# HuiGuanLab/Lite-MKD

Hardware: AMD Instinct MI355X
Metric: episodes/sec (5-way 5-shot, 8x224^2 frames) (higher is better)
Workload: dtype f32

## Files before the change

include/lmkd.h:

```cpp
#ifndef LMKD_H
#define LMKD_H
#ifdef __cplusplus
extern "C" {
#endif

int lmkd_abi_version(void);
const char* lmkd_last_error(void);
int lmkd_device_check(int device);
int lmkd_set_activation_dtype(int mode);
int lmkd_get_activation_dtype(void);

int lmkd_gemm_f32(char layA, char layB, int M, int N, int K, float alpha, const float* A, long lda, long sA,
                  const float* B, long ldb, long sB, float beta, float* C, long ldc, long sC, const float* bias,
                  int relu, int batch, void* stream);
int lmkd_gemm_set_mode(int mode);
int lmkd_gemm_set_tile(int t);
long lmkd_gemm_ticket_words(void);
int lmkd_gemm_f32_splitk(char layA, char layB, int M, int N, int K, float alpha, const float* A, long lda, long sA,
                         const float* B, long ldb, long sB, float beta, float* C, long ldc, long sC, const float* bias,
                         int relu, int batch, void* workspace, long ws_bytes, unsigned* tickets, void* stream);

long lmkd_conv2d_packed_weight_elems(int Cout, int Cin, int Cs, int KH, int KW, int mode);
int lmkd_conv2d_pack_weights(const float* w_oihw, float* wp, int Cout, int Cin, int Cs, int KH, int KW, int mode ,
                             void* stream);
// ... 5 lines not shown
  const void* x_words;
  const void* dy_words;
  void* out_words;
  const void* ref_words;
  int flags;
} lmkd_amax_desc;
#define LMKD_AMAX_FENCED 1
int lmkd_h2_fence_eval(const void* const* words, void* const* refs, int n, int* flags, void* stream);
long lmkd_conv_h2_fallbacks(void);
int lmkd_amax(const float* x, long n, void* word, void* stream);
long lmkd_amax_words(void);
long lmkd_conv2d_plane_elems(int ncols, int Kp);
long lmkd_conv_h2_launches(void);
int lmkd_conv2d_repack_multi(const float* const* ws, void* const* wfs, const int* dims, int n, void* stream);
int lmkd_conv2d_split_weights(const float* wp, void* wf, int ncols, int Kp, void* stream);
int lmkd_conv_get_compute_dtype(void);
int lmkd_conv_set_wgrad_planes(int on);
int lmkd_conv_set_patch(int on);
int lmkd_conv_set_stem_patch(int on);
int lmkd_conv_set_s2_patch(int on);
int lmkd_conv_set_wgrad_win16(int on);
int lmkd_conv_set_wgrad_stem(int on);
int lmkd_conv_set_wgrad_window(int on);
int lmkd_conv_set_patch16(int on);
int lmkd_conv_set_persistent(int on);
int lmkd_conv_set_xcd_mode(int mode);
int lmkd_conv_set_tile(int id);
int lmkd_conv2d_fwd(const float* x, const float* wp_fwd, float* y, float* stat_partial, int N, int H, int W, int Cs, int Cout,
                    int KH, int KW, int stride, int pad, void* stream);
int lmkd_conv2d_fwd_pre(const float* x_raw, const float* pre_stats, const float* wp_fwd, float* y, float* stat_partial, int N, int H,
                        int W, int Cs, int Cout, int KH, int KW, int stride, int pad, void* stream);
int lmkd_conv2d_fwd_bn(const float* x, const float* wp_fwd, float* y, const float* bn_stats, const float* res , int relu,
                       int N, int H, int W, int Cs, int Cout, int KH, int KW, int stride, int pad, void* stream,
                       const lmkd_amax_desc* amax );
int lmkd_conv2d_bwd_data(const float* dy, const float* wp_dgrad, float* dx, int N, int H, int W, int Cin, int Cout, int KH, int KW,
                         int stride, int pad, int accumulate, void* stream);
int lmkd_conv2d_bwd_data_bn_tiles(int N, int H, int W, int Cin, int Cout, int KH, int KW, int stride, int pad);
int lmkd_conv2d_bwd_data_bn(const float* dy, const float* wp_dgrad, float* dx, const float* bn_x, const float* bn_stats, float* part,
                            int N, int H, int W, int Cin, int Cout, int KH, int KW, int stride, int pad, void* stream);
long lmkd_conv2d_bwd_weight_workspace(int N, int H, int W, int Cs, int Cout, int KH, int KW, int stride, int pad);
int lmkd_conv2d_bwd_weight(const float* x, const float* dy, float* dw_oihw, float* workspace, long ws_bytes, int N, int H, int W,
                           int Cs, int Cin, int Cout, int KH, int KW, int stride, int pad, void* stream);
int lmkd_conv2d_bwd_weight_pre(const float* x_raw, const float* pre_stats, const float* dy, float* dw_oihw, float* workspace,
                               long ws_bytes, int N, int H, int W, int Cs, int Cin, int Cout, int KH, int KW, int stride, int pad,
                               void* stream);

// ... 182 lines not shown
```

lite-mkd_amd/csrc/conv.hip:

```cpp
#include "gemm_core.h"
#include <atomic>
#include <mutex>

struct ConvGemmArgs {
  const float* src;
  const float* wpk;
  float* out;
  float* stat_partial;
  int N, Hs, Ws, Cs;
  int Hr, Wr, rows_per_class, tiles_per_class;
  int sh;
  int Ho, Wo, Co, omul;
  int Kp, cps, nclass;
  int n_rt, n_ct, xcd_mode;
  int taps_pm1;
  int grid_step;
  int grid_total;
  int same;
  int halo;
  int accum;
  const float* ep_stats;
  const float* ep_res;
  int ep_relu;
  const float* pre_stats;
// ... 1362 lines not shown
}
extern "C" int lmkd_conv2d_bwd_data_bn(const float* dy, const float* wd, float* dx, const float* bn_x, const float* bn_stats, float* part,
                                       int N, int H, int W, int Cin, int Cout, int KH, int KW, int stride, int pad, void* stream) {
  LMKD_REQUIRE(dy && wd && dx && bn_x && bn_stats && part, "lmkd_conv2d_bwd_data_bn: null pointer");
  LMKD_REQUIRE(aligned16(dy) && aligned16(wd) && aligned16(bn_x) && aligned16(bn_stats), "lmkd_conv2d_bwd_data_bn: operands must be 16-byte aligned");
  ConvGemmArgs a;
  if (const int rc = bwd_data_args(a, dy, wd, dx, N, H, W, Cin, Cout, KH, KW, stride, pad, 0)) return rc;
  a.bnb_x = bn_x; a.bnb_stats = bn_stats; a.stat_partial = part;
  const ConvPlan p = plan_dgrad(a);
  LMKD_REQUIRE(p.bnb_form, "lmkd_conv2d_bwd_data_bn: this launch has no fused form (lmkd_conv2d_bwd_data_bn_tiles returned 0)");
  return launch_conv(a, p, (hipStream_t)stream);
}

static int g_wgrad_planes = 1;
extern "C" int lmkd_conv_set_wgrad_planes(int on) { g_wgrad_planes = on ? 1 : 0; return LMKD_OK; }
static int g_wgrad_win16 = 1;
extern "C" int lmkd_conv_set_wgrad_win16(int on) { g_wgrad_win16 = on ? 1 : 0; return LMKD_OK; }
static int g_wgrad_window = 1;
extern "C" int lmkd_conv_set_wgrad_window(int on) { g_wgrad_window = on < 0 ? 0 : on; return LMKD_OK; }
static inline bool wgrad_win_eligible(int W, int Cs, int Cout, int KH, int KW, int stride, int pad) {
  return g_wgrad_window && g_wgrad_planes && conv_planes() && KH == 3 && KW == 3 && stride == 1 && pad == 1 &&
         Cs % 32 == 0 && 32 + 2 * (W + 1) <= 256;
}
static void wgrad_win_plan(int Mpix, int W, int Cs, int Cout, int* cob, int* splits, int* steps_per_split) {
  *cob = Cout >= 128 ? 4 : 2;
  const int tiles = cdiv(Cout, 32 * *cob) * (Cs / 32);
  const int steps = cdiv(Mpix, LMKD_BK);
  const int warm = cdiv(2 * (W + 1), LMKD_BK);
  const int resident = 256 * ((conv_nprod() >= 6 && *cob == 2) ? 2 : 8 / *cob);
  int sp = g_wgrad_window > 1 ? cdiv(g_wgrad_window, tiles)
                              : std::max((int)(((long)resident * steps + 19600L * 4 / *cob) / (39200L * 4 / *cob)), cdiv(128, tiles));
  const int cap = std::max(1, steps / (12 * warm));
  if (sp > cap) sp = cap;
  *steps_per_split = cdiv(steps, sp);
  *splits = cdiv(steps, *steps_per_split);
}

static void wgrad_plan(int Mpix, int Cout, int Kp, int* splits, int* steps_per_split, int* bm, int* bn, bool planes = false) {
  *bm = Cout <= 64 ? 64 : 128;
  *bn = (Kp % 128 == 0 && Kp >= 1024) ? 128 : 64;
  int per_cu = (*bm == 128 && *bn == 128) ? 2 : ((*bm == 64 && *bn == 64) ? 4 : 3);
  if (planes) {
    if (*bm == 64 && *bn == 128) *bn = 64;
    const int npl = conv_nprod() == 1 ? 1 : 3;
    const long lds = 1L * npl * LMKD_BK * ((*bm * 2 + 64) + (*bn * 2 + 64));
    per_cu = (int)(160 * 1024 / lds);
    if (per_cu > 4) per_cu = 4;
    if (per_cu < 1) per_cu = 1;
  }
  const int tiles = cdiv(Cout, *bm) * cdiv(Kp, *bn);
  const int steps = cdiv(Mpix, LMKD_BK);
  const int slots = 256 * per_cu;
  int best_sp = 1;
  double best_cost = 1e30;
// ... 8 lines not shown
    if (cost < best_cost) { best_cost = cost; best_sp = sp; }
  }
  if (planes && *bm == 64 && *bn == 64 && best_sp < cdiv(steps, 64)) best_sp = cdiv(steps, 64);
  *steps_per_split = cdiv(steps, best_sp);
  *splits = cdiv(steps, *steps_per_split);
}

static int g_wgrad_stem = 1;
extern "C" int lmkd_conv_set_wgrad_stem(int on) { g_wgrad_stem = on ? 1 : 0; return LMKD_OK; }
static int stem_wgrad_plan(int N, int H, int W, int Cs, int Cout, int KH, int KW, int stride, int pad, int* G) {
  if (!g_wgrad_stem || !g_wgrad_planes || conv_nprod(g_lmkd_act_bf16) < 6 || Cs != 4 || Cout != 64 || KH != 7 || KW != 7 || stride != 2 || pad != 3) return 0;
  const int Ho = conv_out(H, KH, stride, pad), Wo = conv_out(W, KW, stride, pad);
  if (Wo < 17 || Wo > 128 || W > 2 * Wo || Ho < 1) return 0;
  const int units = N * cdiv(Ho, 2);
  int g = std::max(1, 2048 / (2 * Wo));
  g = std::min(g, std::max(1, units / 256));
  *G = g;
  return cdiv(units, g);
}

enum class WgFam : unsigned char {
  Stem,
  Win16,
  Win,
  Planes,
  Tile,
};
struct WgradPlan {
  WgFam fam;
  bool pre, act16, smallc;
  int nprod;
  int bm, bn;
  int cob;
  int G;
  int splits, splits0, sps0, sps1, seg_pix0;
  int xcd;
  int grid;
  long need;
  long ws;
};

static long wgrad_workspace(int N, int H, int W, int Cs, int Cout, int KH, int KW, int stride, int pad) {
  const int Ho = conv_out(H, KH, stride, pad), Wo = conv_out(W, KW, stride, pad);
  const int Kp = KH * kw_padded(Cs, KW) * Cs;
  int G, splits, sps, bm, bn;
  if (const int slabs = stem_wgrad_plan(N, H, W, Cs, Cout, KH, KW, stride, pad, &G)) return (long)slabs * Cout * Kp * sizeof(float);
  wgrad_plan(N * Ho * Wo, Cout, Kp, &splits, &sps, &bm, &bn, conv_planes() && g_wgrad_planes);
  if (wgrad_win_eligible(W, Cs, Cout, KH, KW, stride, pad)) {
    int cob, wsplits, wsps;
    wgrad_win_plan(N * Ho * Wo, W, Cs, Cout, &cob, &wsplits, &wsps);
    splits = std::max(splits, wsplits);
  }
  return (long)splits * Cout * Kp * sizeof(float);
}

static WgradPlan plan_wgrad(int N, int H, int W, int Cs, int Cout, int KH, int KW, int stride, int pad, int seg_n0, bool pre, bool maxima) {
  WgradPlan p;
  memset(&p, 0, sizeof(p));
  const bool act16 = g_lmkd_act_bf16;
  const int Ho = conv_out(H, KH, stride, pad), Wo = conv_out(W, KW, stride, pad);
  const int Kp = KH * kw_padded(Cs, KW) * Cs, Mpix = N * Ho * Wo;
  p.pre = pre; p.act16 = act16; p.smallc = Cs == 4;
  p.ws = wgrad_workspace(N, H, W, Cs, Cout, KH, KW, stride, pad);
  if (seg_n0)
    p.ws = std::max(p.ws, wgrad_workspace(seg_n0, H, W, Cs, Cout, KH, KW, stride, pad) + wgrad_workspace(N - seg_n0, H, W, Cs, Cout, KH, KW, stride, pad));
  p.seg_pix0 = seg_n0 ? seg_n0 * Ho * Wo : Mpix;
  if (const int slabs = stem_wgrad_plan(N, H, W, Cs, Cout, KH, KW, stride, pad, &p.G)) {
    p.fam = WgFam::Stem;
    p.nprod = conv_nprod(false, maxima);
    p.splits = p.grid = slabs;
  } else if (wgrad_win_eligible(W, Cs, Cout, KH, KW, stride, pad)) {
    const bool w16 = g_wgrad_win16 && conv_nprod(act16) >= 6;
    p.fam = w16 ? WgFam::Win16 : WgFam::Win;
    p.nprod = w16 ? conv_nprod(false, maxima) : conv_nprod(act16);
    wgrad_win_plan(Mpix, W, Cs, Cout, &p.cob, &p.splits, &p.sps0);
    p.splits0 = p.splits;
    if (seg_n0) {
      int sp1, cob1;
      wgrad_win_plan(p.seg_pix0, W, Cs, Cout, &p.cob, &p.splits0, &p.sps0);
      wgrad_win_plan(Mpix - p.seg_pix0, W, Cs, Cout, &cob1, &sp1, &p.sps1);
      p.splits = p.splits0 + sp1;
    }
    p.grid = 8 * cdiv(p.splits, 8) * cdiv(Cout, 32 * p.cob) * (Cs / 32);
  } else {
    const bool planes = conv_planes() && g_wgrad_planes;
    p.fam = planes ? WgFam::Planes : WgFam::Tile;
    p.nprod = planes ? conv_nprod(act16, maxima && !p.smallc && !pre) : (conv_nprod() == 1 ? 1 : 0);
    wgrad_plan(Mpix, Cout, Kp, &p.splits, &p.sps0, &p.bm, &p.bn, planes);
    p.splits0 = p.splits;
    if (seg_n0) {
      int sp1, bm1, bn1;
      wgrad_plan(p.seg_pix0, Cout, Kp, &p.splits0, &p.sps0, &p.bm, &p.bn, planes);
      wgrad_plan(Mpix - p.seg_pix0, Cout, Kp, &sp1, &p.sps1, &bm1, &bn1, planes);
      p.splits = p.splits0 + sp1;
    }
    p.xcd = (g_xcd_mode != 0 && g_xcd_mode != 1 && p.splits >= 32) ? 1 : 0;
    p.grid = (p.xcd ? 8 * cdiv(p.splits, 8) : p.splits) * cdiv(Cout, p.bm) * cdiv(Kp, p.bn);
  }
  p.need = (long)p.splits * Cout * Kp * sizeof(float);
  return p;
}

template <int NPROD, int D, int RLC>
static void launch_stem_wgrad(const StemWgradArgs& w, dim3 grid, size_t lds, hipStream_t s) {
  lds_attr_once<stem_wgrad_kernel<NPROD, D, RLC>>(160 * 1024);
  hipLaunchKernelGGL((stem_wgrad_kernel<NPROD, D, RLC>), grid, dim3(512), lds, s, w);
}
template <int NPROD>
static void launch_stem_wgrad(const StemWgradArgs& w, dim3 grid, size_t lds, hipStream_t s) {
  const bool deep = cdiv(2 * w.Wo, 32) >= 6;
  if (deep && w.RL == 1856) launch_stem_wgrad<NPROD, 6, 1856>(w, grid, lds, s);
  else if (deep) launch_stem_wgrad<NPROD, 6, 0>(w, grid, lds, s);
  else launch_stem_wgrad<NPROD, 2, 0>(w, grid, lds, s);
}
template <int COB>
static void launch_wgrad_win(const WgradWinArgs& w, const WgradPlan& p, bool big, hipStream_t s) {
  const dim3 grid(p.grid);
  if (p.fam == WgFam::Win16) {
    constexpr int JW = COB == 2 ? 1 : 2;
    constexpr int NT = 64 * COB * (2 / JW);
    with_nprod<3, 6, 9>(p.nprod, [&](auto np) {
      if (big && p.pre) hipLaunchKernelGGL((conv_wgrad_win16_kernel<COB, np, 256, true, 9, JW>), grid, dim3(NT), 0, s, w);
      else if (big) hipLaunchKernelGGL((conv_wgrad_win16_kernel<COB, np, 256, false, 9, JW>), grid, dim3(NT), 0, s, w);
      else if (p.pre) hipLaunchKernelGGL((conv_wgrad_win16_kernel<COB, np, 128, true, 9, JW>), grid, dim3(NT), 0, s, w);
      else hipLaunchKernelGGL((conv_wgrad_win16_kernel<COB, np, 128, false, 9, JW>), grid, dim3(NT), 0, s, w);
    });
    return;
  }
  auto go = [&](auto np, auto a16, auto pre) {
    constexpr int NPROD = decltype(np)::value;
    constexpr bool A16 = decltype(a16)::value, PRE = decltype(pre)::value;
    constexpr int TPW = (COB == 2 && NPROD != 1) ? 5 : 9;
    constexpr int NT = 64 * COB * ((9 + TPW - 1) / TPW);
    if (big) hipLaunchKernelGGL((conv_wgrad_win_kernel<COB, NPROD, A16, 256, PRE, TPW>), grid, dim3(NT), 0, s, w);
    else hipLaunchKernelGGL((conv_wgrad_win_kernel<COB, NPROD, A16, 128, PRE, TPW>), grid, dim3(NT), 0, s, w);
  };
  using T = std::true_type;
  using F = std::false_type;
  if (p.act16) go(std::integral_constant<int, 1>{}, T{}, F{});
  else with_nprod<1, 6, 9>(p.nprod, [&](auto np) { if (p.pre) go(np, F{}, T{}); else go(np, F{}, F{}); });
// ... 44 lines not shown
  LMKD_REQUIRE(ws_bytes >= p.need, "lmkd_conv2d_bwd_weight: workspace too small");
  hipStream_t s = (hipStream_t)stream;
  if (p.fam == WgFam::Stem) {
    LMKD_REQUIRE((long)Mpix * 64 * 4 < 0xffffffe0L && (long)N * H * W * 16 < 0xffffffe0L, "lmkd_conv2d_bwd_weight: tensor too large for 32-bit byte offsets");
    StemWgradArgs w;
    memset(&w, 0, sizeof(w));
    w.dy = dy; w.x = x; w.slab = workspace;
    w.h2_xw = amax_x; w.h2_dyw = amax_dy;
    w.N = N; w.H = H; w.W = W; w.Ho = Ho; w.Wo = Wo;
    w.upi = cdiv(Ho, 2); w.units = N * w.upi; w.G = p.G; w.slabs = p.splits;
    w.RL = 16 * Wo + 64;
    const size_t lds = (size_t)2 * 10 * 3 * w.RL + 2 * 3 * STEM_WG_APLANE;
    with_nprod<3, 6, 9>(p.nprod, [&](auto np) { launch_stem_wgrad<np>(w, dim3(p.grid), lds, s); });
    LMKD_CHECK_LAUNCH("stem_wgrad_kernel");
    if (Kp <= 256) {
      hipLaunchKernelGGL(wgrad_reduce_stem_kernel, dim3(Cout), dim3(256, 4), 0, s, (const float*)workspace, dw_oihw, p.splits, Cout, Cin, Cs, KH, KW,
                         KWp, Kp, accumulate);
    } else {
      launch_wgrad_reduce((const float*)workspace, dw_oihw, p.splits, Cout, Cin, Cs, KH, KW, KWp, Kp, accumulate, s);
    }
    LMKD_CHECK_LAUNCH("wgrad_reduce_kernel");
    return LMKD_OK;
  }
  if (p.fam == WgFam::Win16 || p.fam == WgFam::Win) {
    LMKD_REQUIRE((long)Mpix * std::max(Cs, Cout) * 4 < 2147483647L, "lmkd_conv2d_bwd_weight: tensor too large for 32-bit byte offsets");
    WgradWinArgs w;
    memset(&w, 0, sizeof(w));
    w.dy = dy; w.x = x; w.slab = workspace; w.pre_stats = pre_stats;
    w.h2_xw = amax_x; w.h2_dyw = amax_dy;
    w.N = N; w.H = H; w.W = W; w.Cs = Cs; w.Co = Cout; w.Kp = Kp; w.Mpix = Mpix;
    w.steps_total = cdiv(Mpix, LMKD_BK);
    w.splits = p.splits; w.steps_per_split = p.sps0;
    w.seg_pix0 = p.seg_pix0; w.seg_splits0 = p.splits0; w.sps1 = p.sps1;
    w.n_ct = cdiv(Cout, 32 * p.cob); w.n_it = Cs / 32;
    w.div_hw = make_fastdiv(H * W); w.div_w = make_fastdiv(W);
    const bool big = 32 + 2 * (W + 1) > 128;
    if (p.cob == 4) launch_wgrad_win<4>(w, p, big, s);
    else launch_wgrad_win<2>(w, p, big, s);
    LMKD_CHECK_LAUNCH("conv_wgrad_win_kernel");
    launch_wgrad_reduce((const float*)workspace, dw_oihw, p.splits, Cout, Cin, Cs, KH, KW, KWp, Kp, accumulate, s);
    LMKD_CHECK_LAUNCH("wgrad_reduce_kernel");
    return LMKD_OK;
  }
  WgradArgs a;
  memset(&a, 0, sizeof(a));
  a.dy = dy; a.x = x; a.slab = workspace; a.pre_stats = pre_stats;
  a.h2_xw = amax_x; a.h2_dyw = amax_dy;
  a.N = N; a.Hs = H; a.Ws = W; a.Cs = Cs;
  a.Ho = Ho; a.Wo = Wo; a.Co = Cout;
  a.stride = stride; a.pad = pad; a.KH = KH; a.KW = KW; a.KWp = KWp;
  a.Kp = Kp; a.Mpix = Mpix;
  a.steps_per_split = p.sps0;
  a.seg_pix0 = p.seg_pix0; a.seg_splits0 = p.splits0; a.sps1 = p.sps1;
  a.steps_total = cdiv(Mpix, LMKD_BK);
  a.div_hw = make_fastdiv(Ho * Wo); a.div_w = make_fastdiv(Wo);
  a.n_mt = cdiv(Cout, p.bm); a.n_jt = cdiv(Kp, p.bn); a.splits = p.splits;
  a.xcd_mode = p.xcd;
  const int bm = p.bm, bn = p.bn;
  LMKD_REQUIRE(!smallc || (bm == 64 && bn == 64), "lmkd_conv2d_bwd_weight: padded-stem path expects Cout <= 64");
// ... 39 lines not shown
extern "C" int lmkd_conv2d_bwd_weight_acc(const float* x, const float* pre_stats, const float* dy, float* dw_oihw, float* workspace,
                                          long ws_bytes, int N, int H, int W, int Cs, int Cin, int Cout, int KH, int KW, int stride,
                                          int pad, void* stream) {
  return conv2d_bwd_weight_impl(x, pre_stats, dy, dw_oihw, workspace, ws_bytes, N, H, W, Cs, Cin, Cout, KH, KW, stride, pad, stream, 1);
}


extern "C" int lmkd_conv2d_bwd_weight_seg(const float* x, const float* pre_stats, const float* dy, float* dw_oihw, float* workspace, long ws_bytes,
                                          int N, int H, int W, int Cs, int Cin, int Cout, int KH, int KW, int stride, int pad, int accumulate,
                                          int seg_n0, void* stream, const lmkd_amax_desc* amax) {
  return conv2d_bwd_weight_impl(x, pre_stats, dy, dw_oihw, workspace, ws_bytes, N, H, W, Cs, Cin, Cout, KH, KW, stride, pad, stream, accumulate, seg_n0, amax);
}

extern "C" int lmkd_conv2d_plan(int kind, int N, int H, int W, int Cs, int Cin, int Cout, int KH, int KW, int stride, int pad,
                                int* info) {
  LMKD_REQUIRE(info && kind >= 0 && kind <= 2, "lmkd_conv2d_plan: kind must be 0 (forward), 1 (data gradient) or 2 (weight gradient)");
  LMKD_REQUIRE(N > 0 && H > 0 && W > 0 && Cout > 0 && KH > 0 && KW > 0 && stride > 0, "lmkd_conv2d_plan: bad shape");
  if (kind == 2) {
    const WgradPlan p = plan_wgrad(N, H, W, Cs, Cout, KH, KW, stride, pad, 0, false, false);
    info[1] = p.xcd; info[2] = p.splits; info[3] = p.grid;
    switch (p.fam) {
      case WgFam::Stem: info[0] = 14; info[4] = 2; break;
      case WgFam::Win16:
      case WgFam::Win: info[0] = p.cob == 4 ? 5 : 6; info[1] = 1; info[4] = 1; break;
      default: info[0] = (p.bm == 128 && p.bn == 128) ? 1 : (p.bm == 128 ? 2 : (p.bn == 128 ? 4 : 3)); info[4] = 0; break;
    }
    return LMKD_OK;
  }
  ConvGemmArgs a;
  if (kind == 0) fwd_geometry(a, N, H, W, Cs, Cout, KH, KW, stride, pad, 0);
  else dgrad_geometry(a, N, H, W, Cin, Cout, KH, KW, stride, pad, 0);
  const ConvPlan p = kind == 0 ? plan_fwd(a, KH, KW, pad) : plan_dgrad(a);
  info[0] = p.tile; info[1] = p.xcd; info[2] = p.nclass; info[3] = p.grid;
  info[4] = p.fam == ConvFam::Stem ? 2 : (p.fam == ConvFam::Patch || p.fam == ConvFam::Patch16 || p.fam == ConvFam::Patch1p ? 1 : 0);
  return LMKD_OK;
}
```

lite-mkd_amd/csrc/wgrad_win.h:

```cpp
#pragma once

struct WgradWinArgs {
  const float* dy;
  const float* x;
  float* slab;
  const float* pre_stats;
  int N, H, W, Cs, Co, Kp;
  int Mpix, steps_total, steps_per_split, splits;
  int n_ct, n_it;
  int seg_pix0, seg_splits0, sps1;
  FastDiv div_hw, div_w;
  const unsigned* h2_xw;
  const unsigned* h2_dyw;
};
template <int COB, int NPROD, bool ACT16, int R, bool PRE = false, int TPW = 9>
__global__ __launch_bounds__(64 * COB * ((9 + TPW - 1) / TPW)) void conv_wgrad_win_kernel(WgradWinArgs a) {
  constexpr int NPL = NPROD == 1 ? 1 : 3;
  static_assert(!ACT16 || (NPROD == 1 && !PRE), "bf16 tensors: one plane, no store-side arithmetic");
  constexpr int THREADS = 64 * COB * ((9 + TPW - 1) / TPW), BM = 32 * COB;
  constexpr int LDA = BM * 2 + 64, A_PLANE = LMKD_BK * LDA;
  constexpr int LDX = 64, X_PLANE = (R + 1) * LDX;
  constexpr int ESZ = ACT16 ? 2 : 4, EPL = ACT16 ? 8 : 4;
  constexpr int A_LPR = BM / EPL, A_RPP = THREADS / A_LPR, A_NI = (LMKD_BK + A_RPP - 1) / A_RPP;
  constexpr int X_LPR = 32 / EPL, X_RPP = THREADS / X_LPR, X_NI = (LMKD_BK + X_RPP - 1) / X_RPP;
  static_assert(THREADS % A_LPR == 0 && THREADS % X_LPR == 0 && (LDA / 64) % 2 == 1, "tile layout");
  __shared__ __attribute__((aligned(16))) unsigned char s_dy[NPL * A_PLANE];
  __shared__ __attribute__((aligned(16))) unsigned char s_x[NPL * X_PLANE];
  __shared__ __attribute__((aligned(16))) unsigned s_adr[2][9 * LMKD_BK];
  const int tid = threadIdx.x, lane = tid & 63, wave = tid >> 6;
  const int tiles = a.n_ct * a.n_it;
// ... 144 lines not shown
            c = __builtin_amdgcn_mfma_f32_32x32x16_bf16(fa[g][1], fb[0], c, 0, 0, 0);
            c = __builtin_amdgcn_mfma_f32_32x32x16_bf16(fa[g][0], fb[0], c, 0, 0, 0);
          }
        }
        acc[ti] = c;
      }
      __syncthreads();
    }
  }

  float* C = a.slab + (long)z * a.Co * a.Kp;
#pragma unroll
  for (int ti = 0; ti < TPW; ++ti) {
    if (9 % TPW != 0 && tap0 + ti >= 9) break;
    const int col = (tap0 + ti) * a.Cs + ci0 + (lane & 31);
#pragma unroll
    for (int e = 0; e < 16; ++e) {
      const int row = co0 + cw * 32 + acc_row(e, lane);
      if (row < a.Co) C[(long)row * a.Kp + col] = acc[ti][e];
    }
  }
}

template <int COB, int NPROD, int R, bool PRE = false, int TPW = 9, int JW = 2>
__global__ __launch_bounds__(64 * COB * ((9 + TPW - 1) / TPW) * (2 / JW), JW == 2 ? 2 : 3) void conv_wgrad_win16_kernel(WgradWinArgs a) {
  static_assert(JW == 2 || (JW == 1 && TPW == 9), "the channel-block split exists for nine taps per wave");
  static_assert(NPROD == 6 || NPROD == 9 || NPROD == 3, "three bf16 planes (6 / 9 products) or two fp16 planes (3 products: conv_patch16.h)");
  constexpr int NPL = NPROD == 3 ? 2 : 3;
  constexpr int THREADS = 64 * COB * ((9 + TPW - 1) / TPW) * (2 / JW), BM = 32 * COB;
  constexpr int LDA = BM * 2 + 32, A_PLANE = LMKD_BK * LDA;
  constexpr int LDX = 64, X_PLANE = (R + 1) * LDX;
  constexpr int A_LPR = BM / 4, A_RPP = THREADS / A_LPR, A_NI = (LMKD_BK + A_RPP - 1) / A_RPP;
  constexpr int X_LPR = 8, X_RPP = THREADS / X_LPR, X_NI = (LMKD_BK + X_RPP - 1) / X_RPP;
  static_assert(THREADS % A_LPR == 0 && THREADS % X_LPR == 0 && (LDA / 32) % 2 == 1, "tile layout");
  __shared__ __attribute__((aligned(16))) unsigned char s_dy[NPL * A_PLANE];
  __shared__ __attribute__((aligned(16))) unsigned char s_x[NPL * X_PLANE];
  __shared__ __attribute__((aligned(16))) unsigned s_adr[2][9 * LMKD_BK];
  const int tid = threadIdx.x, lane = tid & 63, wave = tid >> 6;
  const int tiles = a.n_ct * a.n_it;
  const int xj = blockIdx.x >> 3;
  const int z = (blockIdx.x & 7) + 8 * (xj / tiles);
  if (z >= a.splits) return;
  const int tz = xj - (xj / tiles) * tiles;
  const int co0 = (tz % a.n_ct) * BM, ci0 = (tz / a.n_ct) * 32;
  const WinSlab sl = win_slab(z, a.Mpix, a.steps_per_split, a.seg_pix0, a.seg_splits0, a.sps1);
  const int nk = sl.nk, kend = sl.kend;
  const int halo = a.W + 1;

  const __amdgpu_buffer_rsrc_t rs_dy = x3_rsrc(a.dy, (long)a.Mpix * a.Co * 4);
  const __amdgpu_buffer_rsrc_t rs_x = x3_rsrc(a.x, (long)a.Mpix * a.Cs * 4);
  const int a_c = (tid % A_LPR) * 4, a_r = tid / A_LPR;
  const bool a_cin = co0 + a_c < a.Co;
  const int x_c = (tid % X_LPR) * 4, x_r = tid / X_LPR;
  u32x4 ra[A_NI], rx[X_NI];
  unsigned x_ok = 0;
  float h2_sx = 1.f, h2_sdy = 1.f;
  if constexpr (NPROD == 3) {
    h2_sx = h2_scale(amax_read(a.h2_xw, sl.seg));
    h2_sdy = h2_scale(amax_read(a.h2_dyw, sl.seg));
  }
  float4 psc = float4(), psh = float4();
  if (PRE) {
    psc = *reinterpret_cast<const float4*>(a.pre_stats + (long)sl.seg * 5 * a.Cs + 2 * a.Cs + ci0 + x_c);
    psh = *reinterpret_cast<const float4*>(a.pre_stats + (long)sl.seg * 5 * a.Cs + 3 * a.Cs + ci0 + x_c);
  }
  auto load_dy = [&](int k0) {
#pragma unroll
    for (int i = 0; i < A_NI; ++i) {
      const int p = k0 + a_r + A_RPP * i;
      ra[i] = __builtin_amdgcn_raw_buffer_load_b128(rs_dy, (a_cin && a_r + A_RPP * i < LMKD_BK && p < kend) ? (unsigned)((p * a.Co + co0 + a_c) * 4) : X3_OOB, 0, 0);
    }
  };
  auto load_x = [&](int q0) {
#pragma unroll
    for (int i = 0; i < X_NI; ++i) {
      const int q = q0 + x_r + X_RPP * i;
      const bool ok = x_r + X_RPP * i < LMKD_BK && q >= 0 && q < a.Mpix;
      rx[i] = __builtin_amdgcn_raw_buffer_load_b128(rs_x, ok ? (unsigned)((q * a.Cs + ci0 + x_c) * 4) : X3_OOB, 0, 0);
      if (PRE) x_ok = ok ? (x_ok | (1u << i)) : (x_ok & ~(1u << i));
    }
  };
  auto as_f4 = [](const u32x4& r) { return make_float4(__uint_as_float(r.x), __uint_as_float(r.y), __uint_as_float(r.z), __uint_as_float(r.w)); };
  auto store_dy = [&]() {
#pragma unroll
    for (int i = 0; i < A_NI; ++i) {
      if (a_r + A_RPP * i >= LMKD_BK) continue;
      if constexpr (NPROD == 3) {
        uint2 p0, p1;
        h2_split4(as_f4(ra[i]), h2_sdy, p0, p1);
        unsigned char* d = s_dy + (a_r + A_RPP * i) * LDA + a_c * 2;
        *reinterpret_cast<uint2*>(d) = p0;
        *reinterpret_cast<uint2*>(d + A_PLANE) = p1;
      } else {
        tr_store4<NPL, LDA, A_PLANE>(s_dy, a_r + A_RPP * i, a_c, as_f4(ra[i]));
      }
    }
  };
  auto store_x = [&](int q0) {
#pragma unroll
    for (int i = 0; i < X_NI; ++i) {
      if (x_r + X_RPP * i >= LMKD_BK) continue;
      const int slot = (q0 + x_r + X_RPP * i) & (R - 1);
      float4 v = as_f4(rx[i]);
      if (PRE && ((x_ok >> i) & 1u)) {
        v.x = fmaxf(fmaf(v.x, psc.x, psh.x), 0.f); v.y = fmaxf(fmaf(v.y, psc.y, psh.y), 0.f);
        v.z = fmaxf(fmaf(v.z, psc.z, psh.z), 0.f); v.w = fmaxf(fmaf(v.w, psc.w, psh.w), 0.f);
      }
      uint2 p0, p1, p2;
      if constexpr (NPROD == 3) h2_split4(v, h2_sx, p0, p1); else x3_split4(v, p0, p1, p2);
      unsigned char* d = s_x + slot * LDX + ((x_c * 2) ^ (((slot >> 2) & 1) << 5));
      *reinterpret_cast<uint2*>(d) = p0;
      *reinterpret_cast<uint2*>(d + X_PLANE) = p1;
      if constexpr (NPL == 3) *reinterpret_cast<uint2*>(d + 2 * X_PLANE) = p2;
    }
  };
  auto fill_adr = [&](unsigned* tab, int k0) {
    for (int e = tid; e < 9 * LMKD_BK; e += THREADS) {
      const int tp = e >> 5, r = e & 31;
      const int p = k0 + r;
      unsigned adr = (unsigned)(R * LDX);
      if (p < kend) {
        const int n = fdiv(p, a.div_hw);
        const int rem = p - n * a.H * a.W;
        const int h = fdiv(rem, a.div_w), w = rem - h * a.W;
        const int dh = tp / 3 - 1, dw = tp - (tp / 3) * 3 - 1;
        if ((unsigned)(h + dh) < (unsigned)a.H && (unsigned)(w + dw) < (unsigned)a.W) {
          const int slot = (p + dh * a.W + dw) & (R - 1);
          adr = (unsigned)(slot * LDX + (((slot >> 2) & 1) << 5));
        }
      }
      tab[tp * LMKD_BK + (r & 15) * 2 + (r >> 4)] = adr;
    }
  };

  const int q4 = lane >> 4, idx = lane & 15;
  const int cw = wave % COB, tap0 = JW == 2 ? (wave / COB) * TPW : 0, j0 = JW == 2 ? 0 : wave / COB;
  const int offA = (4 * q4 + (idx >> 2)) * LDA + (cw * 32 + 4 * (idx & 3)) * 2;
  const unsigned cbx = (unsigned)(8 * (idx & 3));
  f32x4 acc[TPW][2][JW];
#pragma unroll
  for (int t = 0; t < TPW; ++t)
#pragma unroll
    for (int i = 0; i < 2; ++i)
#pragma unroll
      for (int j = 0; j < JW; ++j) acc[t][i][j] = f32x4{0.f, 0.f, 0.f, 0.f};

  if (nk > 0) {
    const int kfirst = sl.kfirst;
    for (int j = tid; j < NPL * LDX / 4; j += THREADS)
      reinterpret_cast<unsigned*>(s_x + (j / (LDX / 4)) * X_PLANE + R * LDX)[j % (LDX / 4)] = 0u;
    for (int q0 = kfirst - halo; q0 < kfirst + halo; q0 += LMKD_BK) {
      load_x(q0);
      store_x(q0);
    }
    fill_adr(s_adr[0], kfirst);
    load_dy(kfirst);
    load_x(kfirst + halo);
    for (int t = 0; t < nk; ++t) {
      const int k0 = kfirst + t * LMKD_BK;
      store_dy();
      store_x(k0 + halo);
      __syncthreads();
      if (t + 1 < nk) {
        load_dy(k0 + LMKD_BK);
        load_x(k0 + LMKD_BK + halo);
        fill_adr(s_adr[(t + 1) & 1], k0 + LMKD_BK);
      }
      bf16x8 fa[2][NPL];
#pragma unroll
      for (int i = 0; i < 2; ++i)
#pragma unroll
        for (int p = 0; p < NPL; ++p) {
          const unsigned char* ap = s_dy + p * A_PLANE + offA + i * 32;
          const s16x4_t lo = __builtin_amdgcn_ds_read_tr16_b64_v4i16((s16x4_t __attribute__((address_space(3)))*)ap);
          const s16x4_t hi = __builtin_amdgcn_ds_read_tr16_b64_v4i16((s16x4_t __attribute__((address_space(3)))*)(ap + 16 * LDA));
          union { s16x4_t s[2]; bf16x8 b; } u;
          u.s[0] = lo; u.s[1] = hi;
          fa[i][p] = u.b;
        }
      if constexpr (NPROD == 3 && JW == 2) {
        static_assert(NPROD != 3 || TPW == 9, "all nine taps per wave");
        auto read_fb = [&](int tp, bf16x8 (&fb)[JW][NPL]) {
          const uint2 a2 = *reinterpret_cast<const uint2*>(&s_adr[t & 1][tp * LMKD_BK + (4 * q4 + (idx >> 2)) * 2]);
#pragma unroll
          for (int j = 0; j < JW; ++j) {
            const unsigned lo_a = (a2.x ^ (unsigned)((j0 + j) << 5)) + cbx, hi_a = (a2.y ^ (unsigned)((j0 + j) << 5)) + cbx;
#pragma unroll
            for (int p = 0; p < NPL; ++p) {
// ... 111 lines not shown
```

lite-mkd_amd/ops.py:

```python
import ctypes
import os
import itertools
import math

import torch

from ._lib import lib
from . import _audit


def _raw_stream(device_index=None):
    return torch._C._cuda_getCurrentRawStream(torch._C._cuda_getDevice() if device_index is None else device_index)


def _stream():
    return ctypes.c_void_p(_raw_stream())


def _p(t):
    if t is None:
        return None
    if _audit.ON:
        _audit.note(t)
    return ctypes.c_void_p(t.data_ptr())
# ... 24 lines not shown


def _f32(x):
    return ctypes.c_float(float(x))


def _empty(shape, like):
    return torch.empty(shape, dtype=torch.float32, device=like.device)


_ACT_DTYPE = [torch.float32]


def set_activation_dtype(name):
    modes = {"fp32": (0, torch.float32), "bf16": (1, torch.bfloat16)}
    if name not in modes:
        raise ValueError(name)
    lib().call("lmkd_set_activation_dtype", modes[name][0])
    _ACT_DTYPE[0] = modes[name][1]


def get_activation_dtype():
    return "bf16" if _ACT_DTYPE[0] is torch.bfloat16 else "fp32"


def _empty_act(shape, like):
    return torch.empty(shape, dtype=_ACT_DTYPE[0], device=like.device)


def gemm(layA, layB, M, N, K, A, lda, B, ldb, C, ldc, alpha=1.0, beta=0.0, bias=None, relu=False,
         batch=1, sA=0, sB=0, sC=0, A_off=0, B_off=0, C_off=0, split_k=None):
    _chk(A, B, C, bias)
    es = 4
    if _audit.ON:
        for t in (A, B, C):
            _audit.note(t)
    if GEMM_SPLIT_K if split_k is None else split_k:
        ws, tk = _gemm_workspace(C)
        lib().call("lmkd_gemm_f32_splitk", layA.encode(), layB.encode(), M, N, K, _f32(alpha),
                   ctypes.c_void_p(A.data_ptr() + A_off * es), lda, sA,
                   ctypes.c_void_p(B.data_ptr() + B_off * es), ldb, sB, _f32(beta),
                   ctypes.c_void_p(C.data_ptr() + C_off * es), ldc, sC, _p(bias), int(relu), batch, _p(ws), ws.numel(), _p(tk), _stream())
        return C
    lib().call("lmkd_gemm_f32", layA.encode(), layB.encode(), M, N, K, _f32(alpha),
               ctypes.c_void_p(A.data_ptr() + A_off * es), lda, sA,
               ctypes.c_void_p(B.data_ptr() + B_off * es), ldb, sB, _f32(beta),
# ... 2719 lines not shown
```

lite-mkd_amd/schedule.py:

```python
import contextlib
import dataclasses
import os


_PIPELINE = [False]


@dataclasses.dataclass
class Schedule:
    conv_dtype: str = "fp32x3"
    act_dtype: str = "fp32"
    overlap_trunk_calls: bool = True
    merge_trunk_calls: bool = False
    pipeline_episodes: bool = False
    side_wgrad: bool = True
    sync_wgrad_at_backward_end: bool = False
    teacher_stream: bool = True
    heads_on_two_streams: bool = True
    side_linear_wgrad: bool = True
    direct_param_grad: bool = True
    repack_at_step: bool = True
    fuse_two_head_linear: bool = True
    dgrad_bn_stats: bool = True
    stem_pooled_bwd: bool = True
    pre_in_plane_modes: bool = True
    fuse_pre_all_modes: bool = False
    trx_proj_on_conv: bool = False
    gemm_split_k: bool = False

    @classmethod
    def bench(cls, **over):
        kw = dict(merge_trunk_calls=True, pipeline_episodes=True)
        kw.update(over)
        return cls(**kw)

    @classmethod
    def two_call(cls, **over):
        return cls(**over)

    @classmethod
    def serial(cls, **over):
        kw = dict(overlap_trunk_calls=False, merge_trunk_calls=False, side_wgrad=False, sync_wgrad_at_backward_end=True, teacher_stream=False,
                  heads_on_two_streams=False, side_linear_wgrad=False, direct_param_grad=False, repack_at_step=False, pipeline_episodes=False)
        kw.update(over)
        return cls(**kw)

    @classmethod
    def from_env(cls, env=None, **over):
        env = os.environ if env is None else env
        names = {"overlap_trunk_calls": "LMKD_OVERLAP", "merge_trunk_calls": "LMKD_MERGE", "pipeline_episodes": "LMKD_PIPELINE", "side_wgrad": "LMKD_SIDE_WGRAD",
                 "sync_wgrad_at_backward_end": "LMKD_SYNC_WG", "teacher_stream": "LMKD_TEACHER_STREAM", "heads_on_two_streams": "LMKD_HEADS2",
                 "side_linear_wgrad": "LMKD_SIDE_LINEAR", "direct_param_grad": "LMKD_DIRECT_GRAD", "repack_at_step": "LMKD_REPACK",
                 "fuse_two_head_linear": "LMKD_FC_FUSED", "dgrad_bn_stats": "LMKD_DGRAD_BN", "stem_pooled_bwd": "LMKD_STEM_POOLED",
                 "pre_in_plane_modes": "LMKD_PRE_X3", "fuse_pre_all_modes": "LMKD_FUSE_PRE", "trx_proj_on_conv": "LMKD_TRX_CONV",
                 "gemm_split_k": "LMKD_GEMM_SPLIT"}
        s = cls.bench(**over)
        for field, var in names.items():
            if var in env and field not in over:
                setattr(s, field, env[var] == "1")
        return s

    _WHERE = {
        "overlap_trunk_calls": ("model.backbone.resnet", "OVERLAP_TRUNK_CALLS"), "merge_trunk_calls": ("model.backbone.resnet", "MERGE_TRUNK_CALLS"),
        "side_wgrad": ("ops", "SIDE_WGRAD"), "sync_wgrad_at_backward_end": ("ops", "SYNC_WGRAD_AT_BACKWARD_END"),
        "teacher_stream": ("trainloop", "TEACHER_STREAM"), "heads_on_two_streams": ("ops", "HEADS_ON_TWO_STREAMS"),
        "side_linear_wgrad": ("ops", "SIDE_LINEAR_WGRAD"), "direct_param_grad": ("ops", "DIRECT_PARAM_GRAD"),
        "repack_at_step": ("trainloop", "REPACK_AT_STEP"), "fuse_two_head_linear": ("ops", "FUSE_TWO_HEAD_LINEAR"),
        "dgrad_bn_stats": ("ops", "DGRAD_BN_STATS"), "stem_pooled_bwd": ("ops", "STEM_POOLED_BWD"),
        "pre_in_plane_modes": ("ops", "PRE_IN_PLANE_MODES"), "fuse_pre_all_modes": ("ops", "FUSE_PRE_ALL_MODES"),
        "trx_proj_on_conv": ("ops", "TRX_PROJ_ON_CONV"), "gemm_split_k": ("ops", "GEMM_SPLIT_K"),
    }

    def _targets(self):
        import importlib
        pkg = __name__.rsplit(".", 1)[0]
        for field, (mod, attr) in self._WHERE.items():
            yield field, importlib.import_module(pkg + "." + mod), attr

    def apply(self, arithmetic=True):
        from . import ops
        for field, mod, attr in self._targets():
            setattr(mod, attr, bool(getattr(self, field)))
        _PIPELINE[0] = bool(self.pipeline_episodes)
        if arithmetic:
            ops.set_conv_compute_dtype(self.conv_dtype)
            ops.set_activation_dtype(self.act_dtype)
        return self

    @classmethod
    def current(cls):
        from . import ops
        s = cls(conv_dtype=ops.get_conv_compute_dtype(), act_dtype=ops.get_activation_dtype(), pipeline_episodes=_PIPELINE[0])
        for field, mod, attr in s._targets():
            setattr(s, field, bool(getattr(mod, attr)))
        return s

    @contextlib.contextmanager
    def applied(self):
        from . import ops
        prev = Schedule.current()
        ops.join_all_streams()
        self.apply()
        try:
            yield self
        finally:
            ops.join_all_streams()
# ... 2 lines not shown
```

Before: 50.76.

## Add stride-2 sliding-window wgrad kernel for 3x3 convolutions

Extends the windowed weight-gradient kernel to 3x3 stride-2 pad-1 convolutions. Input pixels are split into four parity classes and kept in separate shared-memory rings, so each output pixel's taps index into these rings instead of falling back to the generic planes/tile wgrad path. The change adds the plan, workspace sizing and launch dispatch, plus a schedule flag that is on by default. It adds LDS usage and extra address arithmetic, and it excludes the square Cs==Cout>=128 case.

```diff
diff --git a/include/lmkd.h b/include/lmkd.h
--- a/include/lmkd.h
+++ b/include/lmkd.h
@@ -51,6 +51,7 @@
 int lmkd_conv_set_wgrad_win16(int on);
 int lmkd_conv_set_wgrad_stem(int on);
 int lmkd_conv_set_wgrad_window(int on);
+int lmkd_conv_set_wgrad_window_s2(int on);
 int lmkd_conv_set_patch16(int on);
 int lmkd_conv_set_persistent(int on);
 int lmkd_conv_set_xcd_mode(int mode);
diff --git a/lite-mkd_amd/csrc/conv.hip b/lite-mkd_amd/csrc/conv.hip
--- a/lite-mkd_amd/csrc/conv.hip
+++ b/lite-mkd_amd/csrc/conv.hip
@@ -1408,14 +1408,23 @@
   return g_wgrad_window && g_wgrad_planes && conv_planes() && KH == 3 && KW == 3 && stride == 1 && pad == 1 &&
          Cs % 32 == 0 && 32 + 2 * (W + 1) <= 256;
 }
-static void wgrad_win_plan(int Mpix, int W, int Cs, int Cout, int* cob, int* splits, int* steps_per_split) {
+static int g_wgrad_window_s2 = 0;
+extern "C" int lmkd_conv_set_wgrad_window_s2(int on) { g_wgrad_window_s2 = on ? 1 : 0; return LMKD_OK; }
+static inline bool wgrad_win_s2_eligible(int N, int H, int W, int Cs, int Cout, int KH, int KW, int stride, int pad) {
+  return g_wgrad_window_s2 && g_wgrad_window && g_wgrad_planes && g_wgrad_win16 && conv_nprod(g_lmkd_act_bf16) >= 6 && KH == 3 && KW == 3 &&
+         stride == 2 && pad == 1 && H % 2 == 0 && W % 2 == 0 && Cs % 32 == 0 && Cout % 32 == 0 && 32 + W / 2 + 1 <= 128 &&
+         !(Cs == Cout && Cs >= 128) &&
+         (long)N * H * W * Cs * 4 < 2147483647L;
+}
+static void wgrad_win_plan(int Mpix, int W, int Cs, int Cout, int* cob, int* splits, int* steps_per_split, int stride = 1) {
   *cob = Cout >= 128 ? 4 : 2;
   const int tiles = cdiv(Cout, 32 * *cob) * (Cs / 32);
   const int steps = cdiv(Mpix, LMKD_BK);
-  const int warm = cdiv(2 * (W + 1), LMKD_BK);
+  const int warm = cdiv((stride == 2 ? 1 : 2) * (W + 1), LMKD_BK);
   const int resident = 256 * ((conv_nprod() >= 6 && *cob == 2) ? 2 : 8 / *cob);
+  const long per_round = (stride == 2 ? 19600L : 39200L) * 4 / *cob;
   int sp = g_wgrad_window > 1 ? cdiv(g_wgrad_window, tiles)
-                              : std::max((int)(((long)resident * steps + 19600L * 4 / *cob) / (39200L * 4 / *cob)), cdiv(128, tiles));
+                              : std::max((int)(((long)resident * steps + per_round / 2) / per_round), cdiv(128, tiles));
   const int cap = std::max(1, steps / (12 * warm));
   if (sp > cap) sp = cap;
   *steps_per_split = cdiv(steps, sp);
@@ -1470,6 +1479,7 @@
 enum class WgFam : unsigned char {
   Stem,
   Win16,
+  Win16S2,
   Win,
   Planes,
   Tile,
@@ -1497,6 +1507,10 @@
   if (wgrad_win_eligible(W, Cs, Cout, KH, KW, stride, pad)) {
     int cob, wsplits, wsps;
     wgrad_win_plan(N * Ho * Wo, W, Cs, Cout, &cob, &wsplits, &wsps);
+    splits = std::max(splits, wsplits);
+  } else if (wgrad_win_s2_eligible(N, H, W, Cs, Cout, KH, KW, stride, pad)) {
+    int cob, wsplits, wsps;
+    wgrad_win_plan(N * Ho * Wo, Wo, Cs, Cout, &cob, &wsplits, &wsps, 2);
     splits = std::max(splits, wsplits);
   }
   return (long)splits * Cout * Kp * sizeof(float);
@@ -1530,6 +1544,18 @@
       p.splits = p.splits0 + sp1;
     }
     p.grid = 8 * cdiv(p.splits, 8) * cdiv(Cout, 32 * p.cob) * (Cs / 32);
+  } else if (!pre && wgrad_win_s2_eligible(N, H, W, Cs, Cout, KH, KW, stride, pad)) {
+    p.fam = WgFam::Win16S2;
+    p.nprod = conv_nprod(false, maxima);
+    wgrad_win_plan(Mpix, Wo, Cs, Cout, &p.cob, &p.splits, &p.sps0, 2);
+    p.splits0 = p.splits;
+    if (seg_n0) {
+      int sp1, cob1;
+      wgrad_win_plan(p.seg_pix0, Wo, Cs, Cout, &p.cob, &p.splits0, &p.sps0, 2);
+      wgrad_win_plan(Mpix - p.seg_pix0, Wo, Cs, Cout, &cob1, &sp1, &p.sps1, 2);
+      p.splits = p.splits0 + sp1;
+    }
+    p.grid = 8 * cdiv(p.splits, 8) * cdiv(Cout, 32 * p.cob) * (Cs / 32);
   } else {
     const bool planes = conv_planes() && g_wgrad_planes;
     p.fam = planes ? WgFam::Planes : WgFam::Tile;
@@ -1564,6 +1590,14 @@
 template <int COB>
 static void launch_wgrad_win(const WgradWinArgs& w, const WgradPlan& p, bool big, hipStream_t s) {
   const dim3 grid(p.grid);
+  if (p.fam == WgFam::Win16S2) {
+    constexpr int JW = COB == 2 ? 1 : 2;
+    with_nprod<3, 6, 9>(p.nprod, [&](auto np) {
+      if (big) hipLaunchKernelGGL((conv_wgrad_win16_kernel<COB, np, 128, false, 9, JW, 2>), grid, dim3(256), 0, s, w);
+      else hipLaunchKernelGGL((conv_wgrad_win16_kernel<COB, np, 64, false, 9, JW, 2>), grid, dim3(256), 0, s, w);
+    });
+    return;
+  }
   if (p.fam == WgFam::Win16) {
     constexpr int JW = COB == 2 ? 1 : 2;
     constexpr int NT = 64 * COB * (2 / JW);
@@ -1654,19 +1688,21 @@
     LMKD_CHECK_LAUNCH("wgrad_reduce_kernel");
     return LMKD_OK;
   }
-  if (p.fam == WgFam::Win16 || p.fam == WgFam::Win) {
+  if (p.fam == WgFam::Win16 || p.fam == WgFam::Win16S2 || p.fam == WgFam::Win) {
+    const bool s2 = p.fam == WgFam::Win16S2;
     LMKD_REQUIRE((long)Mpix * std::max(Cs, Cout) * 4 < 2147483647L, "lmkd_conv2d_bwd_weight: tensor too large for 32-bit byte offsets");
     WgradWinArgs w;
     memset(&w, 0, sizeof(w));
     w.dy = dy; w.x = x; w.slab = workspace; w.pre_stats = pre_stats;
     w.h2_xw = amax_x; w.h2_dyw = amax_dy;
     w.N = N; w.H = H; w.W = W; w.Cs = Cs; w.Co = Cout; w.Kp = Kp; w.Mpix = Mpix;
+    w.Ho = Ho; w.Wo = Wo;
     w.steps_total = cdiv(Mpix, LMKD_BK);
     w.splits = p.splits; w.steps_per_split = p.sps0;
     w.seg_pix0 = p.seg_pix0; w.seg_splits0 = p.splits0; w.sps1 = p.sps1;
     w.n_ct = cdiv(Cout, 32 * p.cob); w.n_it = Cs / 32;
-    w.div_hw = make_fastdiv(H * W); w.div_w = make_fastdiv(W);
-    const bool big = 32 + 2 * (W + 1) > 128;
+    w.div_hw = make_fastdiv(Ho * Wo); w.div_w = make_fastdiv(Wo);
+    const bool big = s2 ? 32 + Wo + 1 > 64 : 32 + 2 * (W + 1) > 128;
     if (p.cob == 4) launch_wgrad_win<4>(w, p, big, s);
     else launch_wgrad_win<2>(w, p, big, s);
     LMKD_CHECK_LAUNCH("conv_wgrad_win_kernel");
@@ -1752,6 +1788,7 @@
     switch (p.fam) {
       case WgFam::Stem: info[0] = 14; info[4] = 2; break;
       case WgFam::Win16:
+      case WgFam::Win16S2:
       case WgFam::Win: info[0] = p.cob == 4 ? 5 : 6; info[1] = 1; info[4] = 1; break;
       default: info[0] = (p.bm == 128 && p.bn == 128) ? 1 : (p.bm == 128 ? 2 : (p.bn == 128 ? 4 : 3)); info[4] = 0; break;
     }
diff --git a/lite-mkd_amd/csrc/wgrad_win.h b/lite-mkd_amd/csrc/wgrad_win.h
--- a/lite-mkd_amd/csrc/wgrad_win.h
+++ b/lite-mkd_amd/csrc/wgrad_win.h
@@ -6,6 +6,7 @@
   float* slab;
   const float* pre_stats;
   int N, H, W, Cs, Co, Kp;
+  int Ho, Wo;
   int Mpix, steps_total, steps_per_split, splits;
   int n_ct, n_it;
   int seg_pix0, seg_splits0, sps1;
@@ -196,17 +197,21 @@
   }
 }
 
-template <int COB, int NPROD, int R, bool PRE = false, int TPW = 9, int JW = 2>
+template <int COB, int NPROD, int R, bool PRE = false, int TPW = 9, int JW = 2, int S = 1>
 __global__ __launch_bounds__(64 * COB * ((9 + TPW - 1) / TPW) * (2 / JW), JW == 2 ? 2 : 3) void conv_wgrad_win16_kernel(WgradWinArgs a) {
   static_assert(JW == 2 || (JW == 1 && TPW == 9), "the channel-block split exists for nine taps per wave");
   static_assert(NPROD == 6 || NPROD == 9 || NPROD == 3, "three bf16 planes (6 / 9 products) or two fp16 planes (3 products: conv_patch16.h)");
   constexpr int NPL = NPROD == 3 ? 2 : 3;
   constexpr int THREADS = 64 * COB * ((9 + TPW - 1) / TPW) * (2 / JW), BM = 32 * COB;
   constexpr int LDA = BM * 2 + 32, A_PLANE = LMKD_BK * LDA;
-  constexpr int LDX = 64, X_PLANE = (R + 1) * LDX;
+  constexpr int SLOTS = S == 2 ? 96 + 2 * R : R;
+  constexpr int LDX = 64, X_PLANE = (SLOTS + 1) * LDX;
   constexpr int A_LPR = BM / 4, A_RPP = THREADS / A_LPR, A_NI = (LMKD_BK + A_RPP - 1) / A_RPP;
-  constexpr int X_LPR = 8, X_RPP = THREADS / X_LPR, X_NI = (LMKD_BK + X_RPP - 1) / X_RPP;
+  constexpr int X_LPR = 8, X_RPP = THREADS / X_LPR, X_NI = S == 2 ? 4 : (LMKD_BK + X_RPP - 1) / X_RPP;
   static_assert(THREADS % A_LPR == 0 && THREADS % X_LPR == 0 && (LDA / 32) % 2 == 1, "tile layout");
+  static_assert(S == 1 || (S == 2 && !PRE && X_RPP == LMKD_BK && R >= 64), "stride 2: 256 threads, no BatchNorm loader");
+  auto ring_base = [](int c) { return c == 0 ? 0 : (c == 1 ? 32 : (c == 2 ? 96 : 96 + R)); };
+  auto ring_mask = [](int c) { return c == 0 ? 31 : (c == 1 ? 63 : R - 1); };
   __shared__ __attribute__((aligned(16))) unsigned char s_dy[NPL * A_PLANE];
   __shared__ __attribute__((aligned(16))) unsigned char s_x[NPL * X_PLANE];
   __shared__ __attribute__((aligned(16))) unsigned s_adr[2][9 * LMKD_BK];
@@ -219,10 +224,10 @@
   const int co0 = (tz % a.n_ct) * BM, ci0 = (tz / a.n_ct) * 32;
   const WinSlab sl = win_slab(z, a.Mpix, a.steps_per_split, a.seg_pix0, a.seg_splits0, a.sps1);
   const int nk = sl.nk, kend = sl.kend;
-  const int halo = a.W + 1;
+  const int halo = S == 2 ? a.Wo + 1 : a.W + 1;
 
   const __amdgpu_buffer_rsrc_t rs_dy = x3_rsrc(a.dy, (long)a.Mpix * a.Co * 4);
-  const __amdgpu_buffer_rsrc_t rs_x = x3_rsrc(a.x, (long)a.Mpix * a.Cs * 4);
+  const __amdgpu_buffer_rsrc_t rs_x = x3_rsrc(a.x, (long)a.N * a.H * a.W * a.Cs * 4);
   const int a_c = (tid % A_LPR) * 4, a_r = tid / A_LPR;
   const bool a_cin = co0 + a_c < a.Co;
   const int x_c = (tid % X_LPR) * 4, x_r = tid / X_LPR;
@@ -246,6 +251,19 @@
     }
   };
   auto load_x = [&](int q0) {
+    if constexpr (S == 2) {
+      const int q = q0 + x_r;
+      const bool ok = q >= 0 && q < a.Mpix;
+      const int qq = ok ? q : 0;
+      const int n = fdiv(qq, a.div_hw);
+      const int rem = qq - n * a.Ho * a.Wo;
+      const int r = fdiv(rem, a.div_w), c = rem - r * a.Wo;
+      const int e00 = ((n * a.H + 2 * r) * a.W + 2 * c) * a.Cs + ci0 + x_c;
+#pragma unroll
+      for (int i = 0; i < 4; ++i)
+        rx[i] = __builtin_amdgcn_raw_buffer_load_b128(rs_x, ok ? (unsigned)((e00 + ((i >> 1) * a.W + (i & 1)) * a.Cs) * 4) : X3_OOB, 0, 0);
+      return;
+    }
 #pragma unroll
     for (int i = 0; i < X_NI; ++i) {
       const int q = q0 + x_r + X_RPP * i;
@@ -273,8 +291,8 @@
   auto store_x = [&](int q0) {
 #pragma unroll
     for (int i = 0; i < X_NI; ++i) {
-      if (x_r + X_RPP * i >= LMKD_BK) continue;
-      const int slot = (q0 + x_r + X_RPP * i) & (R - 1);
+      if (S == 1 && x_r + X_RPP * i >= LMKD_BK) continue;
+      const int slot = S == 2 ? ring_base(i) + ((q0 + x_r) & ring_mask(i)) : ((q0 + x_r + X_RPP * i) & (R - 1));
       float4 v = as_f4(rx[i]);
       if (PRE && ((x_ok >> i) & 1u)) {
         v.x = fmaxf(fmaf(v.x, psc.x, psh.x), 0.f); v.y = fmaxf(fmaf(v.y, psc.y, psh.y), 0.f);
@@ -292,8 +310,18 @@
     for (int e = tid; e < 9 * LMKD_BK; e += THREADS) {
       const int tp = e >> 5, r = e & 31;
       const int p = k0 + r;
-      unsigned adr = (unsigned)(R * LDX);
-      if (p < kend) {
+      unsigned adr = (unsigned)(SLOTS * LDX);
+      if (S == 2 && p < kend) {
+        const int n = fdiv(p, a.div_hw);
+        const int rem = p - n * a.Ho * a.Wo;
+        const int oh = fdiv(rem, a.div_w), ow = rem - oh * a.Wo;
+        const int kh = tp / 3, kw = tp - kh * 3;
+        const int dr = kh == 0, dc = kw == 0, cls = (kh != 1) * 2 + (kw != 1);
+        if (oh >= dr && ow >= dc) {
+          const int slot = ring_base(cls) + ((p - dr * a.Wo - dc) & ring_mask(cls));
+          adr = (unsigned)(slot * LDX + (((slot >> 2) & 1) << 5));
+        }
+      } else if (p < kend) {
         const int n = fdiv(p, a.div_hw);
         const int rem = p - n * a.H * a.W;
         const int h = fdiv(rem, a.div_w), w = rem - h * a.W;
@@ -322,22 +350,24 @@
   if (nk > 0) {
     const int kfirst = sl.kfirst;
     for (int j = tid; j < NPL * LDX / 4; j += THREADS)
-      reinterpret_cast<unsigned*>(s_x + (j / (LDX / 4)) * X_PLANE + R * LDX)[j % (LDX / 4)] = 0u;
-    for (int q0 = kfirst - halo; q0 < kfirst + halo; q0 += LMKD_BK) {
+      reinterpret_cast<unsigned*>(s_x + (j / (LDX / 4)) * X_PLANE + SLOTS * LDX)[j % (LDX / 4)] = 0u;
+    constexpr int FWD = S == 2 ? 0 : 1;
+    for (int q0 = kfirst - halo; q0 < kfirst + FWD * halo; q0 += LMKD_BK) {
       load_x(q0);
       store_x(q0);
     }
+    if (S == 2) __syncthreads();
     fill_adr(s_adr[0], kfirst);
     load_dy(kfirst);
-    load_x(kfirst + halo);
+    load_x(kfirst + FWD * halo);
     for (int t = 0; t < nk; ++t) {
       const int k0 = kfirst + t * LMKD_BK;
       store_dy();
-      store_x(k0 + halo);
+      store_x(k0 + FWD * halo);
       __syncthreads();
       if (t + 1 < nk) {
         load_dy(k0 + LMKD_BK);
-        load_x(k0 + LMKD_BK + halo);
+        load_x(k0 + LMKD_BK + FWD * halo);
         fill_adr(s_adr[(t + 1) & 1], k0 + LMKD_BK);
       }
       bf16x8 fa[2][NPL];
diff --git a/lite-mkd_amd/ops.py b/lite-mkd_amd/ops.py
--- a/lite-mkd_amd/ops.py
+++ b/lite-mkd_amd/ops.py
@@ -70,6 +70,15 @@
 
 def get_activation_dtype():
     return "bf16" if _ACT_DTYPE[0] is torch.bfloat16 else "fp32"
+
+
+WGRAD_WINDOW_S2 = False
+
+
+def set_wgrad_window_s2(on):
+    global WGRAD_WINDOW_S2
+    WGRAD_WINDOW_S2 = bool(on)
+    lib().call("lmkd_conv_set_wgrad_window_s2", int(WGRAD_WINDOW_S2))
 
 
 def _empty_act(shape, like):
diff --git a/lite-mkd_amd/schedule.py b/lite-mkd_amd/schedule.py
--- a/lite-mkd_amd/schedule.py
+++ b/lite-mkd_amd/schedule.py
@@ -27,6 +27,7 @@
     fuse_pre_all_modes: bool = False
     trx_proj_on_conv: bool = False
     gemm_split_k: bool = False
+    wgrad_window_s2: bool = True
 
     @classmethod
     def bench(cls, **over):
@@ -68,7 +69,7 @@
         "repack_at_step": ("trainloop", "REPACK_AT_STEP"), "fuse_two_head_linear": ("ops", "FUSE_TWO_HEAD_LINEAR"),
         "dgrad_bn_stats": ("ops", "DGRAD_BN_STATS"), "stem_pooled_bwd": ("ops", "STEM_POOLED_BWD"),
         "pre_in_plane_modes": ("ops", "PRE_IN_PLANE_MODES"), "fuse_pre_all_modes": ("ops", "FUSE_PRE_ALL_MODES"),
-        "trx_proj_on_conv": ("ops", "TRX_PROJ_ON_CONV"), "gemm_split_k": ("ops", "GEMM_SPLIT_K"),
+        "trx_proj_on_conv": ("ops", "TRX_PROJ_ON_CONV"), "gemm_split_k": ("ops", "GEMM_SPLIT_K"), "wgrad_window_s2": ("ops", "WGRAD_WINDOW_S2"),
     }
 
     def _targets(self):
@@ -82,6 +83,7 @@
         for field, mod, attr in self._targets():
             setattr(mod, attr, bool(getattr(self, field)))
         _PIPELINE[0] = bool(self.pipeline_episodes)
+        ops.set_wgrad_window_s2(self.wgrad_window_s2)
         if arithmetic:
             ops.set_conv_compute_dtype(self.conv_dtype)
             ops.set_activation_dtype(self.act_dtype)
```

After: 50.97 (median of 6 runs). Within noise of the previous version (+0.4%).
